# yandex/pire

Hardware: AMD Instinct MI355X
Metric: scanned GB/s (whole node) + ns/byte, 8-regex glued Scanner, 4KiB strings (higher is better)
Workload: dtype u8

## Files before the change

pire_amd/csrc/slow.hip:

```cpp

#include <hip/hip_runtime.h>

#include <algorithm>
#include <cstdio>
#include <cstdlib>
#include <cstring>
#include <memory>
#include <new>
#include <vector>

#include "internal.h"
#include "walk.h"

namespace pirehip {

struct SlowHost {
	uint32_t states = 0, letters = 0, start = 0, words = 0;
	bool empty = false;
	std::vector<uint8_t> letterOf;
	std::vector<uint32_t> masks;
	std::vector<uint32_t> single;
	std::vector<uint32_t> finals;
	std::vector<uint32_t> jumpPos;
	std::vector<uint32_t> jumps;
	bool wide = false;
	std::vector<uint32_t> pair16;
};

struct SlowDevice {
	int device = -1;
	uint8_t* letterOf = nullptr;
	uint32_t* masks = nullptr;
	uint32_t* single = nullptr;
	uint32_t* finals = nullptr;
	uint32_t* jumpPos = nullptr;
	uint32_t* jumps = nullptr;
	uint32_t* pair16 = nullptr;
};

constexpr uint32_t kSlowNone = 0xFFFFFFFFu;
constexpr uint32_t kSlowMulti = 0xFFFFFFFEu;

}

struct pire_hip_slow_table {
	pirehip::SlowHost host;
	pirehip::SlowDevice devs[pirehip::kMaxDevices];
	std::mutex uploadMutex;
};

namespace pirehip {

struct SlowParams {
	const uint8_t* letterOf;
	const uint32_t* masks;
	const uint32_t* single;
	const uint32_t* finals;
	const uint32_t* jumpPos;
	const uint32_t* jumps;
	const uint32_t* pair16;
	uint32_t* overflow;
	const uint32_t* order;
	uint32_t serpentine;
	uint32_t* scratch;
	uint32_t states, letters, start, words, flags, masksInLds, singleInLds;
	const uint8_t* text;
	const uint64_t* offsets;
	uint64_t n, len, stride;
	uint8_t* outFinal;
	uint32_t* outBits;
	unsigned long long* outCounts;
};

template <int K>
__device__ __forceinline__ void SlowStep(const uint32_t* masks, uint32_t letters, uint32_t (&cur)[K], uint32_t letter)
{
	uint32_t next[K];
#pragma unroll
	for (int k = 0; k < K; ++k)
		next[k] = 0;
#pragma unroll
	for (int w = 0; w < K; ++w) {
		uint32_t bits = cur[w];
		while (bits) {
			const uint32_t s = w * 32 + __builtin_ctz(bits);
			bits &= bits - 1;
			const uint32_t* row = masks + (size_t(s) * letters + letter) * K;
#pragma unroll
			for (int k = 0; k < K; ++k)
				next[k] |= row[k];
		}
	}
#pragma unroll
	for (int k = 0; k < K; ++k)
		cur[k] = next[k];
}

template <int K>
struct SlowLane {
	uint32_t lst[4];
	uint32_t cur[K];
	uint32_t E;
	bool bits;

	__device__ __forceinline__ void Start(uint32_t start, uint32_t states)
	{
		E = states;
		lst[0] = start;
		lst[1] = lst[2] = lst[3] = E;
		bits = false;
#pragma unroll
		for (int k = 0; k < K; ++k)
			cur[k] = 0;
	}
	__device__ __forceinline__ void ListToBits()
	{
#pragma unroll
		for (int k = 0; k < K; ++k)
			cur[k] = 0;
#pragma unroll
		for (int i = 0; i < 4; ++i) {
			const uint32_t s = lst[i];
			if (s != E) {
#pragma unroll
				for (int k = 0; k < K; ++k)
					cur[k] |= (s >> 5) == uint32_t(k) ? (1u << (s & 31)) : 0u;
			}
		}
		bits = true;
	}
	__device__ __forceinline__ void BitsToListIfSmall()
	{
		uint32_t count = 0;
#pragma unroll
		for (int k = 0; k < K; ++k)
			count += __popc(cur[k]);
		if (count > 4)
			return;
		uint32_t n[4] = {E, E, E, E};
		uint32_t used = 0;
#pragma unroll
		for (int k = 0; k < K; ++k) {
			uint32_t b = cur[k];
			while (b) {
				const uint32_t s = uint32_t(k) * 32 + __builtin_ctz(b);
				b &= b - 1;
				n[0] = used == 0 ? s : n[0];
				n[1] = used == 1 ? s : n[1];
				n[2] = used == 2 ? s : n[2];
				n[3] = used == 3 ? s : n[3];
				++used;
			}
		}
#pragma unroll
		for (int i = 0; i < 4; ++i)
			lst[i] = n[i];
		bits = false;
	}
	__device__ __forceinline__ void Step(const uint32_t* masks, const uint2* single, uint32_t letters, uint32_t letter)
	{
		if (!bits) {
			uint32_t n[4], extra = 0, extras = 0, multi = 0;
#pragma unroll
			for (int i = 0; i < 4; ++i) {
				const uint2 r = single[__umul24(lst[i], letters) + letter];
				n[i] = r.x;
				multi |= r.x;
				const bool has = int32_t(r.y) >= 0;
				extra = has ? r.y : extra;
				extras += has ? 1u : 0u;
			}
			uint32_t overflow = multi >> 31;
			if (__any(extras != 0)) {
				overflow |= uint32_t(extras > 1);
				uint32_t placed = uint32_t(extras != 1);
#pragma unroll
				for (int j = 0; j < 4; ++j) {
					const uint32_t take = uint32_t(n[j] == E) & (placed ^ 1u);
					n[j] = take ? extra : n[j];
					placed |= take;
				}
				overflow |= placed ^ 1u;
			}
			if (!overflow) {
#pragma unroll
				for (int i = 0; i < 4; ++i)
					lst[i] = n[i];
				return;
			}
			ListToBits();
		}
		SlowStep<K>(masks, letters, cur, letter);
		BitsToListIfSmall();
	}
	__device__ __forceinline__ bool Final(const uint32_t* finals) const
	{
		bool fin = false;
		if (bits) {
#pragma unroll
			for (int k = 0; k < K; ++k)
				fin = fin || (cur[k] & finals[k]) != 0;
		} else {
#pragma unroll
			for (int i = 0; i < 4; ++i)
				fin = fin || (lst[i] != E && ((finals[lst[i] >> 5] >> (lst[i] & 31)) & 1u));
		}
		return fin;
	}
};

template <int K>
__global__ __launch_bounds__(1024) void SlowScanKernel(SlowParams p)
{
	extern __shared__ __attribute__((aligned(16))) uint8_t lds[];
	uint8_t* ldsLetter = lds;
	uint32_t* ldsSingle = reinterpret_cast<uint32_t*>(lds + 272);
	const uint32_t entries = p.states * p.letters;
	const uint32_t singleEntries = (p.states + 1) * p.letters;
	uint32_t* ldsMasks = ldsSingle + (p.singleInLds ? 2 * singleEntries : 0);
	for (uint32_t i = threadIdx.x; i < 264; i += blockDim.x)
		ldsLetter[i] = p.letterOf[i];
	if (p.singleInLds)
		for (uint32_t i = threadIdx.x; i < 2 * singleEntries; i += blockDim.x)
			ldsSingle[i] = p.single[i];
	const uint32_t maskWords = entries * K;
	if (p.masksInLds)
		for (uint32_t i = threadIdx.x; i < maskWords; i += blockDim.x)
			ldsMasks[i] = p.masks[i];
	__syncthreads();
	const uint32_t* masks = p.masksInLds ? ldsMasks : p.masks;
	const uint2* single = reinterpret_cast<const uint2*>(p.singleInLds ? ldsSingle : p.single);

	const uint64_t stride = uint64_t(gridDim.x) * blockDim.x;
	unsigned long long finals = 0, strings = 0;
	const uint64_t todo = p.overflow ? p.overflow[0] : p.n;
	for (uint64_t k = uint64_t(blockIdx.x) * blockDim.x + threadIdx.x; k < todo; k += stride) {
		const uint64_t s = p.overflow ? p.overflow[1 + k] : k;
		uint64_t b, e;
		if (p.offsets) {
			b = p.offsets[s];
			e = p.offsets[s + 1];
		} else {
			b = s * p.stride;
			e = b + p.len;
		}
		SlowLane<K> lane;
		lane.Start(p.start, p.states);
		if (p.flags & PIRE_HIP_RUN_BEGIN)
			lane.Step(masks, single, p.letters, ldsLetter[kBeginMark]);
		const uint8_t* ptr = p.text + b;
		const uint8_t* end = p.text + e;
		for (; ptr < end && (reinterpret_cast<uintptr_t>(ptr) & 15); ++ptr)
			lane.Step(masks, single, p.letters, ldsLetter[*ptr]);
		uint4 ahead = ptr + 16 <= end ? *reinterpret_cast<const uint4*>(ptr) : uint4{0, 0, 0, 0};
		for (; ptr + 16 <= end; ptr += 16) {
			uint4 v = ahead;
			if (ptr + 32 <= end)
				ahead = *reinterpret_cast<const uint4*>(ptr + 16);
#pragma unroll 1
			for (int i = 0; i < 16; ++i) {
				lane.Step(masks, single, p.letters, ldsLetter[v.x & 0xFF]);
				NextByte(v);
			}
		}
		for (; ptr < end; ++ptr)
			lane.Step(masks, single, p.letters, ldsLetter[*ptr]);
		if (p.flags & PIRE_HIP_RUN_END)
			lane.Step(masks, single, p.letters, ldsLetter[kEndMark]);
		const bool fin = lane.Final(p.finals);
		if (p.outFinal)
			p.outFinal[s] = fin ? 1 : 0;
		if (p.outBits) {
			if (!lane.bits)
				lane.ListToBits();
#pragma unroll
			for (int k = 0; k < K; ++k)
				if (uint32_t(k) < p.words)
					p.outBits[s * p.words + k] = lane.cur[k];
		}
		finals += fin ? 1 : 0;
		strings += 1;
	}
	if (p.outCounts) {
		for (int off = 32; off > 0; off >>= 1) {
			finals += __shfl_down(finals, off);
			strings += __shfl_down(strings, off);
		}
		if ((threadIdx.x & 63) == 0 && strings) {
			atomicAdd(&p.outCounts[0], finals);
			atomicAdd(&p.outCounts[1], strings);
		}
	}
}

constexpr int kListSlots = 16;
constexpr uint32_t kListMulti = 0x7FFFu;
constexpr uint32_t kListMaxRows = 16383;

typedef const __attribute__((address_space(3))) uint32_t* LdsWordPtr;

template <int T>
__device__ __forceinline__ void ListStepT(uint32_t tabBase, uint32_t letter4, uint32_t (&lst)[kListSlots], bool& ovf)
{
	constexpr int N = 4 * T;
	uint32_t r[N];
	uint32_t sumHi = 0;
	const uint32_t base = letter4 + tabBase;
#pragma unroll
	for (int i = 0; i < N; ++i) {
		uint32_t addr;
		asm("v_mad_u32_u16 %0, %1, 1, %2" : "=v"(addr) : "v"(lst[i]), "v"(base));
		r[i] = *reinterpret_cast<LdsWordPtr>(static_cast<uintptr_t>(addr));
		sumHi += r[i] >> 16;
	}
	const bool spawn = sumHi != 0;
	const uint32_t extra = sumHi & 0x7FFFu;
	bool over = sumHi >= (0x8000u | kListMulti);
	if (N == kListSlots)
		over = over || (spawn && (r[N - 1] & 0xFFFFu) != 0);
	if (__any(over)) {
		ovf = ovf || over;
#pragma unroll
		for (int i = 0; i < N; ++i)
			r[i] = over ? 0u : r[i];
	}
	const bool shift = spawn && !ovf;
	if (N < kListSlots)
		lst[N] = shift ? r[N - 1] : 0u;
#pragma unroll
	for (int i = N - 1; i > 0; --i)
		lst[i] = shift ? r[i - 1] : r[i];
	lst[0] = shift ? extra << 2 : r[0];
}

__device__ __forceinline__ uint32_t ListTop(const uint32_t (&lst)[kListSlots])
{
	uint32_t top = 1;
#pragma unroll
	for (int g = 1; g < kListSlots / 4; ++g)
		top = __any((lst[4 * g] | lst[4 * g + 1] | lst[4 * g + 2] | lst[4 * g + 3]) != 0) ? uint32_t(g + 1) : top;
	return top;
}

__device__ __forceinline__ void ListStepTop(uint32_t tabBase, uint32_t letter4, uint32_t (&lst)[kListSlots], bool& ovf, uint32_t& top)
{
	switch (top) {
	case 1:
		ListStepT<1>(tabBase, letter4, lst, ovf);
		top = __any(lst[4] != 0) ? 2u : 1u;
		break;
	case 2:
		ListStepT<2>(tabBase, letter4, lst, ovf);
		top = __any(lst[8] != 0) ? 3u : __any((lst[4] | lst[5] | lst[6] | lst[7]) != 0) ? 2u : 1u;
		break;
	case 3:
		ListStepT<3>(tabBase, letter4, lst, ovf);
		top = __any(lst[12] != 0) ? 4u : __any((lst[8] | lst[9] | lst[10] | lst[11]) != 0) ? 3u : 2u;
		break;
	default:
		ListStepT<4>(tabBase, letter4, lst, ovf);
		top = __any((lst[12] | lst[13] | lst[14] | lst[15]) != 0) ? 4u : 3u;
		break;
	}
}

__device__ __forceinline__ void ListStep(uint32_t tabBase, uint32_t letter4, uint32_t (&lst)[kListSlots], bool& ovf)
{
	ListStepT<kListSlots / 4>(tabBase, letter4, lst, ovf);
}

__global__ __launch_bounds__(1024) void SlowListKernel(SlowParams p)
{
	extern __shared__ __attribute__((aligned(16))) uint8_t lds[];
	uint8_t* ldsLetter = lds;
	uint32_t* tab = reinterpret_cast<uint32_t*>(lds + 1056 + 16);
	const uint32_t tabBase = 1056 + 16;
	uint32_t* ldsLetter4 = reinterpret_cast<uint32_t*>(lds);
	const uint32_t entries = (p.states + 1) * p.letters;
	for (uint32_t i = threadIdx.x; i < 264; i += blockDim.x)
		ldsLetter4[i] = 4u * p.letterOf[i];
	for (uint32_t i = threadIdx.x; i < entries; i += blockDim.x)
		tab[i] = p.pair16[i];
	__syncthreads();
	(void)ldsLetter;
	const uint64_t stride = uint64_t(gridDim.x) * blockDim.x;
	unsigned long long finals = 0, strings = 0;
	for (uint64_t pass = 0; pass * stride < p.n; ++pass) {
		const uint64_t k = OrderedIndex(pass, uint64_t(blockIdx.x) * blockDim.x + threadIdx.x, stride, p.serpentine != 0);
		if (k >= p.n)
			continue;
		const uint64_t s = p.order ? p.order[k] : k;
		uint64_t b, e;
		if (p.offsets) {
			b = p.offsets[s];
			e = p.offsets[s + 1];
		} else {
#if defined(PIRE_EXP) && PIRE_EXP == 21
			b = (s & 63) * p.stride;
#else
			b = s * p.stride;
#endif
			e = b + p.len;
		}
		uint32_t lst[kListSlots];
		lst[0] = (p.start + 1) * p.letters * 4;
#pragma unroll
		for (int i = 1; i < kListSlots; ++i)
			lst[i] = 0;
		bool ovf = false;
		if (p.flags & PIRE_HIP_RUN_BEGIN)
			ListStep(tabBase, ldsLetter4[kBeginMark], lst, ovf);
		const uint8_t* ptr = p.text + b;
		const uint8_t* end = p.text + e;
		for (; ptr < end && (reinterpret_cast<uintptr_t>(ptr) & 15); ++ptr)
			ListStep(tabBase, ldsLetter4[*ptr], lst, ovf);
		uint4 ahead = ptr + 16 <= end ? *reinterpret_cast<const uint4*>(ptr) : uint4{0, 0, 0, 0};
		uint32_t top = ListTop(lst);
		for (; ptr + 16 <= end; ptr += 16) {
			top = __builtin_amdgcn_readfirstlane(top);
			uint4 v = ahead;
			if (ptr + 32 <= end)
				ahead = *reinterpret_cast<const uint4*>(ptr + 16);
#pragma unroll 1
			for (int i = 0; i < 4; ++i) {
				const uint32_t x = v.x;
				ListStepTop(tabBase, ldsLetter4[x & 0xFF], lst, ovf, top);
				ListStepTop(tabBase, ldsLetter4[(x >> 8) & 0xFF], lst, ovf, top);
				ListStepTop(tabBase, ldsLetter4[(x >> 16) & 0xFF], lst, ovf, top);
				ListStepTop(tabBase, ldsLetter4[x >> 24], lst, ovf, top);
				v.x = v.y;
				v.y = v.z;
				v.z = v.w;
			}
		}
		for (; ptr < end; ++ptr)
			ListStep(tabBase, ldsLetter4[*ptr], lst, ovf);
		if (p.flags & PIRE_HIP_RUN_END)
			ListStep(tabBase, ldsLetter4[kEndMark], lst, ovf);
		if (ovf) {
			const uint32_t k = atomicAdd(&p.overflow[0], 1u);
			p.overflow[1 + k] = uint32_t(s);
			continue;
		}
		bool fin = false;
#pragma unroll
		for (int i = 0; i < kListSlots; ++i) {
			const uint32_t row = (lst[i] & 0xFFFFu) >> 2;
			lst[i] = row ? row / p.letters - 1 : p.states;
			fin = fin || (lst[i] != p.states && ((p.finals[lst[i] >> 5] >> (lst[i] & 31)) & 1u));
		}
		if (p.outFinal)
			p.outFinal[s] = fin ? 1 : 0;
		if (p.outBits) {
			uint32_t* row = p.outBits + s * p.words;
			for (uint32_t w = 0; w < p.words; ++w) {
				uint32_t v = 0;
#pragma unroll
				for (int i = 0; i < kListSlots; ++i)
					v |= (lst[i] != p.states && (lst[i] >> 5) == w) ? 1u << (lst[i] & 31) : 0u;
				row[w] = v;
			}
		}
		finals += fin ? 1 : 0;
		strings += 1;
	}
	if (p.outCounts) {
		for (int off = 32; off > 0; off >>= 1) {
			finals += __shfl_down(finals, off);
			strings += __shfl_down(strings, off);
		}
		if ((threadIdx.x & 63) == 0 && strings) {
			atomicAdd(&p.outCounts[0], finals);
			atomicAdd(&p.outCounts[1], strings);
		}
	}
}

template <bool SETS_LDS>
__device__ __forceinline__ void WideSync()
{
	if (SETS_LDS)
		__builtin_amdgcn_fence(__ATOMIC_SEQ_CST, "workgroup");
	else
		__builtin_amdgcn_fence(__ATOMIC_SEQ_CST, "agent");
	__builtin_amdgcn_wave_barrier();
}
template <bool SETS_LDS>
__device__ __forceinline__ uint32_t WideLoad(const uint32_t* q)
{
	if (SETS_LDS)
		return *q;
	return __hip_atomic_load(q, __ATOMIC_RELAXED, __HIP_MEMORY_SCOPE_AGENT);
}
template <bool SETS_LDS>
__device__ __forceinline__ void WideStore(uint32_t* q, uint32_t v)
{
	if (SETS_LDS)
		*q = v;
	else
		__hip_atomic_store(q, v, __ATOMIC_RELAXED, __HIP_MEMORY_SCOPE_AGENT);
}

struct WideTables {
	const uint32_t* pos;
	const uint32_t* jumps;
};

template <bool SETS_LDS>
__device__ __forceinline__ void WideStep(const SlowParams& p, const WideTables& T, uint32_t*& cur, uint32_t*& next,
                                         uint32_t letter, uint32_t lane)
{
	for (uint32_t w = lane; w < p.words; w += 64)
		WideStore<SETS_LDS>(&next[w], 0u);
	WideSync<SETS_LDS>();
	for (uint32_t w0 = 0; w0 < p.words; w0 += 64) {
		const uint32_t mine = w0 + lane < p.words ? WideLoad<SETS_LDS>(&cur[w0 + lane]) : 0u;
		unsigned long long nz = __ballot(mine != 0);
		while (nz) {
			const int j = __builtin_ctzll(nz);
			nz &= nz - 1;
			uint32_t bits = uint32_t(__builtin_amdgcn_readlane(int(mine), j));
			const uint32_t base = (w0 + uint32_t(j)) * 32;
			while (bits) {
				const uint32_t s = base + uint32_t(__builtin_ctz(bits));
				bits &= bits - 1;
				const uint32_t* pos = T.pos + size_t(s) * p.letters + letter;
				const uint32_t lo = pos[0], hi = pos[1];
				for (uint32_t k = lo + lane; k < hi; k += 64) {
					const uint32_t t = T.jumps[k];
					atomicOr(&next[t >> 5], 1u << (t & 31));
				}
			}
		}
	}
	WideSync<SETS_LDS>();
	uint32_t* tmp = cur;
	cur = next;
	next = tmp;
}

template <bool SETS_LDS>
__global__ __launch_bounds__(1024) void SlowWideKernel(SlowParams p, uint32_t wavesPerBlock, uint32_t posInLds,
                                                       uint32_t jumpsInLds, uint32_t njumps)
{
	extern __shared__ __attribute__((aligned(16))) uint8_t lds[];
	uint8_t* ldsLetter = lds;
	uint32_t* ldsPos = reinterpret_cast<uint32_t*>(lds + 272);
	const uint32_t npos = p.states * p.letters + 1;
	uint32_t* ldsJumps = ldsPos + (posInLds ? npos : 0);
	uint32_t* ldsSets = ldsJumps + (jumpsInLds ? njumps : 0);
	for (uint32_t i = threadIdx.x; i < 264; i += blockDim.x)
		ldsLetter[i] = p.letterOf[i];
	if (posInLds)
		for (uint32_t i = threadIdx.x; i < npos; i += blockDim.x)
			ldsPos[i] = p.jumpPos[i];
	if (jumpsInLds)
		for (uint32_t i = threadIdx.x; i < njumps; i += blockDim.x)
			ldsJumps[i] = p.jumps[i];
	__syncthreads();
	WideTables T;
	T.pos = posInLds ? ldsPos : p.jumpPos;
	T.jumps = jumpsInLds ? ldsJumps : p.jumps;
	const uint32_t lane = threadIdx.x & 63;
	const uint32_t wave = threadIdx.x >> 6;
	const uint64_t gwave = uint64_t(blockIdx.x) * wavesPerBlock + wave;
	uint32_t* setA = SETS_LDS ? ldsSets + size_t(wave) * 2 * p.words : p.scratch + gwave * 2 * p.words;
	uint32_t* setB = setA + p.words;
	unsigned long long finals = 0, strings = 0;
	const uint64_t todo = p.overflow ? p.overflow[0] : p.n;
	for (uint64_t k = gwave; k < todo; k += uint64_t(gridDim.x) * wavesPerBlock) {
		const uint64_t s = p.overflow ? p.overflow[1 + k] : k;
		uint64_t b, e;
		if (p.offsets) {
			b = p.offsets[s];
			e = p.offsets[s + 1];
		} else {
			b = s * p.stride;
			e = b + p.len;
		}
		uint32_t *cur = setA, *next = setB;
		for (uint32_t w = lane; w < p.words; w += 64)
			WideStore<SETS_LDS>(&cur[w], (p.start >> 5) == w ? 1u << (p.start & 31) : 0u);
		WideSync<SETS_LDS>();
		if (p.flags & PIRE_HIP_RUN_BEGIN)
			WideStep<SETS_LDS>(p, T, cur, next, ldsLetter[kBeginMark], lane);
		for (uint64_t i = b; i < e; i += 64) {
			const uint32_t mine = i + lane < e ? p.text[i + lane] : 0u;
			const uint32_t cnt = e - i < 64 ? uint32_t(e - i) : 64u;
			for (uint32_t k = 0; k < cnt; ++k)
				WideStep<SETS_LDS>(p, T, cur, next, ldsLetter[__builtin_amdgcn_readlane(int(mine), int(k))], lane);
		}
		if (p.flags & PIRE_HIP_RUN_END)
			WideStep<SETS_LDS>(p, T, cur, next, ldsLetter[kEndMark], lane);
		bool fin = false;
		for (uint32_t w = lane; w < p.words; w += 64) {
			const uint32_t v = WideLoad<SETS_LDS>(&cur[w]);
			fin = fin || (v & p.finals[w]) != 0;
			if (p.outBits)
				p.outBits[s * p.words + w] = v;
		}
		fin = __any(fin);
		if (p.outFinal && lane == 0)
			p.outFinal[s] = fin ? 1 : 0;
		finals += fin ? 1 : 0;
		strings += 1;
		WideSync<SETS_LDS>();
	}
	if (p.outCounts && lane == 0 && strings) {
		atomicAdd(&p.outCounts[0], finals);
		atomicAdd(&p.outCounts[1], strings);
	}
}

namespace {

size_t Up8(size_t v) { return (v + 7) & ~size_t(7); }

int BadSlow(const char* msg)
{
	SetError(msg);
	return PIRE_HIP_EFORMAT;
}

int BuildSlowHost(const void* blob, size_t len, SlowHost* out)
{
	const uint8_t* p = static_cast<const uint8_t*>(blob);
	if (!p || len < 24 + 24 + 8)
		return BadSlow("EOF reached while reading the SlowScanner header");
	uint32_t hdr[6];
	memcpy(hdr, p, 24);
	if (hdr[0] != 0x45524950u || hdr[2] != 8 || hdr[3] != 16)
		return BadSlow("Serialized regexp incompatible with your system");
	if (hdr[1] != 7 && hdr[1] != 6)
		return BadSlow("You are trying to used an incompatible version of a serialized regexp");
	if (hdr[4] != 3  || hdr[5] != 24)
		return BadSlow("Serialized regexp incompatible with your system");
	uint64_t states, letters, start;
	memcpy(&states, p + 24, 8);
	memcpy(&letters, p + 32, 8);
	memcpy(&start, p + 40, 8);
	size_t pos = 48;
	const bool empty = p[pos] != 0;
	pos += 8;
	SlowHost& h = *out;
	h = SlowHost();
	h.empty = empty;
	if (empty) {
		h.states = 1;
		h.letters = 1;
		h.start = 0;
		h.words = 1;
		h.letterOf.assign(kMaxChar, 0);
		h.masks.assign(1, 0);
		h.single.assign(4, kSlowNone);
		h.single[0] = h.single[2] = 1;
		h.finals.assign(1, 0);
		return PIRE_HIP_OK;
	}
	if (states == 0 || letters == 0 || letters > 256 || states > (1u << 20) || start >= states)
		return BadSlow("Corrupt SlowScanner: bad geometry");
	h.states = uint32_t(states);
	h.letters = uint32_t(letters);
	h.start = uint32_t(start);
	h.words = (h.states + 31) / 32;
	if (len < pos + size_t(kMaxChar) * 8)
		return BadSlow("EOF reached while reading SlowScanner letters");
	h.letterOf.assign(kMaxChar, 0);
	for (uint32_t c = 0; c < kMaxChar; ++c) {
		uint64_t v;
		memcpy(&v, p + pos + size_t(c) * 8, 8);
		if (v >= letters)
			return BadSlow("Corrupt SlowScanner: letter out of range");
		h.letterOf[c] = uint8_t(v);
	}
	pos += size_t(kMaxChar) * 8;
	if (len < pos + Up8(states))
		return BadSlow("EOF reached while reading SlowScanner finals");
	h.finals.assign(h.words, 0);
	for (uint32_t s = 0; s < h.states; ++s)
		if (p[pos + s])
			h.finals[s >> 5] |= 1u << (s & 31);
	pos += Up8(states);
	const size_t npos = size_t(states) * letters + 1;
	if (len < pos + npos * 8)
		return BadSlow("EOF reached while reading SlowScanner jump positions");
	std::vector<uint64_t> jumpPos(npos);
	memcpy(jumpPos.data(), p + pos, npos * 8);
	pos += npos * 8;
	const uint64_t njumps = jumpPos[npos - 1];
	if (len < pos + Up8(size_t(njumps) * 4))
		return BadSlow("EOF reached while reading SlowScanner jumps");
	if (njumps >= (1ull << 32))
		return BadSlow("Corrupt SlowScanner: too many jumps");
	for (size_t i = 0; i + 1 < npos; ++i)
		if (jumpPos[i] > jumpPos[i + 1] || jumpPos[i + 1] > njumps)
			return BadSlow("Corrupt SlowScanner: jump positions not monotone");
	for (uint64_t k = 0; k < njumps; ++k) {
		uint32_t tgt;
		memcpy(&tgt, p + pos + size_t(k) * 4, 4);
		if (tgt >= states)
			return BadSlow("Corrupt SlowScanner: jump target out of range");
	}
	if ((size_t(states) + 1) * letters <= kListMaxRows) {
		h.pair16.assign((size_t(states) + 1) * letters, 0);
		for (size_t i = 0; i + 1 < npos; ++i) {
			const uint32_t self = uint32_t(i / letters);
			uint32_t t0 = kSlowNone, t1 = kSlowNone;
			bool multi = false;
			for (uint64_t k = jumpPos[i]; k < jumpPos[i + 1]; ++k) {
				uint32_t tgt;
				memcpy(&tgt, p + pos + size_t(k) * 4, 4);
				if (t0 == kSlowNone)
					t0 = tgt;
				else if (tgt == t0)
					continue;
				else if (t1 == kSlowNone)
					t1 = tgt;
				else if (tgt != t1)
					multi = true;
			}
			if (t1 != kSlowNone && t0 == self)
				std::swap(t0, t1);
			const auto rowIndex = [&](uint32_t t) { return uint32_t((size_t(t) + 1) * letters); };
			uint32_t& w = h.pair16[letters + i];
			if (multi)
				w = (1u << 31) | (kListMulti << 16);
			else if (t1 != kSlowNone)
				w = (1u << 31) | (rowIndex(t1) << 16) | (rowIndex(t0) * 4);
			else if (t0 != kSlowNone)
				w = rowIndex(t0) * 4;
		}
	}
	h.wide = h.words > 8;
	if (h.wide) {
		h.jumpPos.resize(npos);
		for (size_t i = 0; i < npos; ++i)
			h.jumpPos[i] = uint32_t(jumpPos[i]);
		h.jumps.resize(size_t(njumps));
		memcpy(h.jumps.data(), p + pos, size_t(njumps) * 4);
		return PIRE_HIP_OK;
	}
	h.masks.assign(size_t(states) * letters * h.words, 0);
	for (size_t i = 0; i + 1 < npos; ++i)
		for (uint64_t k = jumpPos[i]; k < jumpPos[i + 1]; ++k) {
			uint32_t tgt;
			memcpy(&tgt, p + pos + size_t(k) * 4, 4);
			h.masks[i * h.words + (tgt >> 5)] |= 1u << (tgt & 31);
		}
	h.single.assign(size_t(states + 1) * letters * 2, kSlowNone);
	for (uint64_t l = 0; l < letters; ++l)
		h.single[(size_t(states) * letters + l) * 2] = uint32_t(states);
	for (size_t i = 0; i + 1 < npos; ++i) {
		uint32_t t0 = kSlowNone, t1 = kSlowNone;
		bool multi = false;
		for (uint64_t k = jumpPos[i]; k < jumpPos[i + 1]; ++k) {
			uint32_t tgt;
			memcpy(&tgt, p + pos + size_t(k) * 4, 4);
			if (t0 == kSlowNone)
				t0 = tgt;
			else if (tgt == t0)
				continue;
			else if (t1 == kSlowNone)
				t1 = tgt;
			else if (tgt != t1)
				multi = true;
		}
		h.single[2 * i] = multi ? kSlowMulti : t0 == kSlowNone ? uint32_t(states) : t0;
		h.single[2 * i + 1] = multi ? kSlowNone : t1;
	}
	return PIRE_HIP_OK;
}

template <class T>
int PutSlow(T** dst, const std::vector<T>& src)
{
	*dst = nullptr;
	hipError_t e = hipMalloc(reinterpret_cast<void**>(dst), std::max<size_t>(src.size() * sizeof(T), 16));
	if (e != hipSuccess)
		return HipFail(e, "hipMalloc(slow table)");
	if (!src.empty()) {
		e = hipMemcpy(*dst, src.data(), src.size() * sizeof(T), hipMemcpyHostToDevice);
		if (e != hipSuccess)
			return HipFail(e, "hipMemcpy(slow table)");
	}
	return PIRE_HIP_OK;
}

void FreeSlowDevice(SlowDevice* d)
{
	if (d->device < 0)
		return;
	if (d->letterOf) (void)hipFree(d->letterOf);
	if (d->masks) (void)hipFree(d->masks);
	if (d->single) (void)hipFree(d->single);
	if (d->finals) (void)hipFree(d->finals);
	if (d->jumpPos) (void)hipFree(d->jumpPos);
	if (d->jumps) (void)hipFree(d->jumps);
	if (d->pair16) (void)hipFree(d->pair16);
	*d = SlowDevice();
}

int DeviceK(uint32_t words)
{
	return words <= 1 ? 1 : words <= 2 ? 2 : words <= 4 ? 4 : words <= 8 ? 8 : 0;
}

int UploadSlow(pire_hip_slow_table* t, SlowDevice* image)
{
	std::lock_guard<std::mutex> lock(t->uploadMutex);
	int dev = -1;
	hipError_t e = hipGetDevice(&dev);
	if (e != hipSuccess)
		return HipFail(e, "hipGetDevice");
	if (dev < 0 || dev >= kMaxDevices) {
		SetError("HIP device ordinal out of range");
		return PIRE_HIP_EUNSUPPORTED;
	}
	if (t->devs[dev].device == dev) {
		*image = t->devs[dev];
		return PIRE_HIP_OK;
	}
	const SlowHost& h = t->host;
	if (h.wide) {
		SlowDevice d;
		int rc;
		if ((rc = PutSlow(&d.letterOf, h.letterOf)) || (rc = PutSlow(&d.finals, h.finals)) ||
		    (rc = PutSlow(&d.jumpPos, h.jumpPos)) || (rc = PutSlow(&d.jumps, h.jumps)) ||
		    (!h.pair16.empty() && (rc = PutSlow(&d.pair16, h.pair16)))) {
			d.device = dev;
			FreeSlowDevice(&d);
			return rc;
		}
		d.device = dev;
		t->devs[dev] = d;
		*image = d;
		return PIRE_HIP_OK;
	}
	const int K = DeviceK(h.words);
	std::vector<uint32_t> masks(size_t(h.states) * h.letters * K, 0), finals(K, 0);
	for (size_t i = 0; i < size_t(h.states) * h.letters; ++i)
		for (uint32_t w = 0; w < h.words; ++w)
			masks[i * K + w] = h.masks[i * h.words + w];
	for (uint32_t w = 0; w < h.words; ++w)
		finals[w] = h.finals[w];
	SlowDevice d;
	int rc;
	if ((rc = PutSlow(&d.letterOf, h.letterOf)) || (rc = PutSlow(&d.masks, masks)) || (rc = PutSlow(&d.single, h.single)) ||
	    (rc = PutSlow(&d.finals, finals)) || (!h.pair16.empty() && (rc = PutSlow(&d.pair16, h.pair16)))) {
		d.device = dev;
		FreeSlowDevice(&d);
		return rc;
	}
	d.device = dev;
	t->devs[dev] = d;
	*image = d;
	return PIRE_HIP_OK;
}

struct SlowGeometry {
	uint32_t states, letters, words, njumps;
	bool listTable;
};

struct SlowGrid {
	uint32_t threads = 0, blocks = 0, ldsBytes = 0;
	uint64_t passes = 0;
};

enum : uint32_t { kSlowFirstList = 0, kSlowFirstScan = 1, kSlowFirstWide = 2 };

struct SlowPlan {
	uint32_t first = 0;
	uint32_t walker = 0;
	uint32_t K = 0;
	uint32_t listTable = 0;
	uint32_t byLength = 0;
	SlowGrid list;
	uint32_t singleInLds = 0, masksInLds = 0;
	uint32_t waves = 0, posInLds = 0, jumpsInLds = 0, setsInLds = 0;
	SlowGrid walk;
};

constexpr size_t kSlowSingleLdsMax = 64 * 1024;
constexpr size_t kSlowTablesLdsMax = 150 * 1024;
constexpr uint64_t kSlowScanBigBatch = 128 * 1024;
constexpr size_t kSlowWideLdsRoom = 158 * 1024 - 272;
constexpr uint32_t kSlowWideWaves = 16;

uint64_t GridPasses(uint64_t n, uint64_t lanes)
{
	return (n + lanes - 1) / lanes;
}

SlowPlan PlanSlow(const SlowGeometry& g, uint64_t n, bool ragged, int cus, const pire_hip_config& c)
{
	SlowPlan plan;
	const bool wide = g.words > 8;
	plan.K = wide ? 0 : uint32_t(DeviceK(g.words));
	plan.listTable = g.listTable ? 1 : 0;
	plan.walker = wide ? kSlowFirstWide : kSlowFirstScan;
	plan.first = g.listTable && n < (1ull << 32) - 1 && !c.slow_no_list ? uint32_t(kSlowFirstList) : plan.walker;
	if (plan.first == kSlowFirstList) {
		plan.byLength = ragged && OrdersByLength(n, c) ? 1 : 0;
		SlowGrid& l = plan.list;
		l.ldsBytes = uint32_t(1056 + 16 + size_t(g.states + 1) * g.letters * 4);
		l.threads = n >= uint64_t(cus) * 2048 ? 1024 : n >= uint64_t(cus) * 512 ? 512 : 256;
		l.blocks = GridBlocks(n, cus, l.threads, l.ldsBytes);
		l.passes = GridPasses(n, uint64_t(l.blocks) * l.threads);
	}
	SlowGrid& w = plan.walk;
	if (!wide) {
		const size_t maskBytes = size_t(g.states) * g.letters * plan.K * 4;
		const size_t singleBytes = size_t(g.states + 1) * g.letters * 8;
		plan.singleInLds = singleBytes <= kSlowSingleLdsMax ? 1 : 0;
		plan.masksInLds = maskBytes + (plan.singleInLds ? singleBytes : 0) <= kSlowTablesLdsMax ? 1 : 0;
		w.ldsBytes = uint32_t(272 + (plan.singleInLds ? singleBytes : 0) + (plan.masksInLds ? maskBytes : 0));
		w.threads = n >= kSlowScanBigBatch ? 1024 : 256;
		w.blocks = GridBlocks(n, cus, w.threads, w.ldsBytes);
		w.passes = GridPasses(n, uint64_t(w.blocks) * w.threads);
		return plan;
	}
	const size_t setBytes = size_t(g.words) * 8;
	uint32_t waves = uint32_t(std::min<size_t>(kSlowWideWaves, kSlowWideLdsRoom / setBytes));
	const bool inLds = waves >= 1 && !c.slow_sets_in_memory;
	if (!inLds)
		waves = kSlowWideWaves;
	size_t room = kSlowWideLdsRoom - (inLds ? waves * setBytes : 0);
	const size_t posBytes = (size_t(g.states) * g.letters + 1) * 4, jumpBytes = size_t(g.njumps) * 4;
	plan.posInLds = posBytes <= room ? 1 : 0;
	if (plan.posInLds)
		room -= posBytes;
	plan.jumpsInLds = plan.posInLds && jumpBytes <= room ? 1 : 0;
	plan.setsInLds = inLds ? 1 : 0;
	plan.waves = waves;
	w.threads = waves * 64;
	w.blocks = uint32_t(std::max<uint64_t>(1, std::min<uint64_t>((n + waves - 1) / waves, uint64_t(cus))));
	w.ldsBytes = uint32_t(272 + (inLds ? waves * setBytes : 0) + (plan.posInLds ? posBytes : 0) + (plan.jumpsInLds ? jumpBytes : 0));
	w.passes = GridPasses(n, uint64_t(w.blocks) * waves);
	return plan;
}

SlowGeometry GeometryOf(const SlowHost& h)
{
	return SlowGeometry{h.states, h.letters, h.words, uint32_t(h.jumps.size()), !h.pair16.empty()};
}

template <int K>
int LaunchSlowK(const SlowParams& p0, const SlowPlan& plan, hipStream_t stream)
{
	SlowParams p = p0;
	p.singleInLds = plan.singleInLds;
	p.masksInLds = plan.masksInLds;
	return Launch(SlowScanKernel<K>, plan.walk.blocks, plan.walk.threads, plan.walk.ldsBytes, stream, "slow kernel launch", p);
}

int LaunchSlowWide(const SlowParams& p0, const SlowPlan& plan, uint32_t njumps, hipStream_t stream)
{
	SlowParams p = p0;
	StreamScratch scratch(stream);
	if (!plan.setsInLds) {
		if (int rc = scratch.Alloc(uint64_t(plan.walk.blocks) * plan.waves * p.words * 8, "hipMallocAsync(slow scanner sets)"))
			return rc;
		p.scratch = scratch.as<uint32_t>();
	}
	return Launch(plan.setsInLds ? SlowWideKernel<true> : SlowWideKernel<false>, plan.walk.blocks, plan.walk.threads, plan.walk.ldsBytes,
	              stream, "slow kernel launch", p, plan.waves, plan.posInLds, plan.jumpsInLds, njumps);
}

template <class Fallback>
int LaunchSlowListThen(const SlowParams& p0, const SlowPlan& plan, hipStream_t stream, Fallback fallback)
{
	SlowParams p = p0;
	StreamScratch list(stream);
	if (int rc = OverflowList(list, p.n, stream, "hipMallocAsync(slow scanner overflow list)", &p.overflow))
		return rc;
	StreamScratch orderScratch(stream);
	p.order = nullptr;
	if (plan.byLength)
		if (int rc = OrderByLength(p.offsets, p.n, stream, orderScratch, &p.order, &p.serpentine))
			return rc;
	if (int rc = Launch(SlowListKernel, plan.list.blocks, plan.list.threads, plan.list.ldsBytes, stream, "slow kernel launch", p))
		return rc;
	if (GetConfig().slow_stats) {
		uint32_t over = 0;
		if (hipStreamSynchronize(stream) == hipSuccess && hipMemcpy(&over, list.get(), 4, hipMemcpyDeviceToHost) == hipSuccess)
			fprintf(stderr, "pire_hip slow: %u of %llu strings left the list kernel for the %s one\n", over,
			        static_cast<unsigned long long>(p.n), p.words > 8 ? "wave-per-string" : "bitset");
	}
	return fallback(p);
}

int RunSlow(const char* who, pire_hip_slow_table* t, const void* text, const uint64_t* offsets, uint64_t n, uint64_t len, uint64_t stride,
            uint32_t flags, uint8_t* outFinal, uint32_t* outBits, uint64_t* outCounts, const FinalSelectOut* sel, void* streamPtr)
{
	if (!t) {
		SetError(sel ? std::string(who) + ": null table" : std::string("null table"));
		return PIRE_HIP_EINVAL;
	}
	const bool onDevice = (flags & PIRE_HIP_RUN_ON_DEVICE) != 0;
	std::optional<FinalSelectStage> pass;
	if (sel) {
		if (int rc = FinalSelectArgsInvalid(who, n, true, *sel))
			return rc;
		pass.emplace(*sel, onDevice);
		if (n == 0)
			return pass->Empty(static_cast<hipStream_t>(streamPtr));
	}
	SlowDevice image;
	if (int rc = UploadSlow(t, &image))
		return rc;
	hipStream_t stream = static_cast<hipStream_t>(streamPtr);
	const SlowHost& h = t->host;
	SlowParams p;
	memset(&p, 0, sizeof(p));
	p.letterOf = image.letterOf;
	p.masks = image.masks;
	p.single = image.single;
	p.finals = image.finals;
	p.jumpPos = image.jumpPos;
	p.jumps = image.jumps;
	p.pair16 = image.pair16;
	p.states = h.states;
	p.letters = h.letters;
	p.start = h.start;
	p.words = h.words;
	p.flags = flags;
	p.n = n;
	p.len = len;
	p.stride = stride;
	if (n == 0)
		return PIRE_HIP_OK;
	int cus = 0;
	if (int rc = DeviceCUs(&cus))
		return rc;
	const SlowPlan plan = PlanSlow(GeometryOf(h), n, offsets != nullptr, cus, GetConfig());
	auto plain = [&](const SlowParams& q) {
		switch (plan.K) {
		case 0: return LaunchSlowWide(q, plan, uint32_t(h.jumps.size()), stream);
		case 1: return LaunchSlowK<1>(q, plan, stream);
		case 2: return LaunchSlowK<2>(q, plan, stream);
		case 4: return LaunchSlowK<4>(q, plan, stream);
		default: return LaunchSlowK<8>(q, plan, stream);
		}
	};
	auto launch = [&](const SlowParams& q) {
		if (plan.first == kSlowFirstList) {
			NoteKernel("slow_list", "pirehip::SlowListKernel");
			return LaunchSlowListThen(q, plan, stream, plain);
		}
		if (plan.first == kSlowFirstWide)
			NoteKernel("slow_wide", "pirehip::SlowWideKernel");
		else
			NoteKernel("slow", plan.K == 1 ? "pirehip::SlowScanKernel<1>" : plan.K == 2 ? "pirehip::SlowScanKernel<2>" :
			                    plan.K == 4 ? "pirehip::SlowScanKernel<4>" : "pirehip::SlowScanKernel<8>");
		return plain(q);
	};
	BatchIO io(stream, onDevice);
	const unsigned long long* dCnt = nullptr;
	int rc = io.Text(text, offsets, n, len, stride, &p.text, &p.offsets);
	if (!rc && outCounts) {
		rc = io.In(reinterpret_cast<const unsigned long long*>(outCounts), 2, &dCnt);
		p.outCounts = const_cast<unsigned long long*>(dCnt);
	}
	if (!rc && (outFinal || pass))
		rc = io.Result(outFinal, n, n, &p.outFinal);
	if (!rc && outBits)
		rc = io.Result(outBits, n * h.words, n * h.words, &p.outBits);
	io.CopyBack(outCounts, dCnt, 16);
	StreamScratch ownFinal(stream);
	if (!rc && pass) {
		if (!p.outFinal) {
			if ((rc = ownFinal.Alloc(size_t(n), "hipMallocAsync(slow scanner final flags)")))
				return rc;
			p.outFinal = ownFinal.as<uint8_t>();
		}
		rc = pass->Results(io, n);
	}
	if (rc || (rc = io.Ready()) || (rc = launch(p)))
		return rc;
	if (pass && (rc = pass->Launch(p.outFinal, n, stream)))
		return rc;
	if ((rc = io.Finish()))
		return rc;
	return pass ? pass->Back() : PIRE_HIP_OK;
}

}
}

using namespace pirehip;

extern "C" {

int pire_hip_slow_table_create(const void* save_blob, size_t len, pire_hip_slow_table** out)
try {
	if (!out) {
		SetError("null out pointer");
		return PIRE_HIP_EINVAL;
	}
	*out = nullptr;
	std::unique_ptr<pire_hip_slow_table> t(new (std::nothrow) pire_hip_slow_table);
	if (!t) {
		SetError("out of memory");
		return PIRE_HIP_ENOMEM;
	}
	if (int rc = BuildSlowHost(save_blob, len, &t->host))
		return rc;
	*out = t.release();
	return PIRE_HIP_OK;
} catch (...) {
	return pirehip::HandleException();
}

void pire_hip_slow_table_destroy(pire_hip_slow_table* t)
{
	if (!t)
		return;
	int cur = -1;
	(void)hipGetDevice(&cur);
	for (int k = 0; k < kMaxDevices; ++k)
		if (t->devs[k].device >= 0) {
			(void)hipSetDevice(k);
			FreeSlowDevice(&t->devs[k]);
		}
	if (cur >= 0)
		(void)hipSetDevice(cur);
	delete t;
}

int pire_hip_slow_table_get_info(const pire_hip_slow_table* t, pire_hip_slow_info* out)
try {
	if (!t || !out) {
		SetError("null argument");
		return PIRE_HIP_EINVAL;
	}
	memset(out, 0, sizeof(*out));
	out->states = t->host.states;
	out->letters = t->host.letters;
	out->start = t->host.start;
	out->words = t->host.words;
	out->empty = t->host.empty ? 1 : 0;
	out->mask_bytes = uint64_t(t->host.masks.size()) * 4;
	return PIRE_HIP_OK;
} catch (...) {
	return pirehip::HandleException();
}

int pire_hip_slow_table_plan(const pire_hip_slow_table* t, uint64_t n, uint32_t ragged, uint32_t cus, uint32_t out[24])
try {
	if (!t || !out) {
		SetError("null argument");
		return PIRE_HIP_EINVAL;
	}
	int units = int(cus);
	if (cus == 0)
		if (int rc = DeviceCUs(&units))
			return rc;
	if (units <= 0) {
		SetError("bad CU count");
		return PIRE_HIP_EINVAL;
	}
	const SlowPlan plan = PlanSlow(GeometryOf(t->host), n, ragged != 0, units, GetConfig());
	const SlowGrid& first = plan.first == kSlowFirstList ? plan.list : plan.walk;
	const auto sat = [](uint64_t v) { return uint32_t(std::min<uint64_t>(v, 0xFFFFFFFFu)); };
	memset(out, 0, 24 * sizeof(uint32_t));
	out[0] = plan.first;
	out[1] = plan.walker;
	out[2] = plan.K;
	out[3] = plan.listTable;
	out[4] = plan.singleInLds;
	out[5] = plan.masksInLds;
	out[6] = first.threads;
	out[7] = first.blocks;
	out[8] = first.ldsBytes;
	out[9] = sat(first.passes);
	out[10] = plan.waves;
	out[11] = plan.posInLds;
	out[12] = plan.jumpsInLds;
	out[13] = plan.setsInLds;
	out[14] = plan.byLength;
	out[15] = plan.walk.threads;
	out[16] = plan.walk.blocks;
	out[17] = plan.walk.ldsBytes;
	out[18] = sat(plan.walk.passes);
	out[19] = uint32_t(units);
	return PIRE_HIP_OK;
} catch (...) {
	return pirehip::HandleException();
}

int pire_hip_slow_run(pire_hip_slow_table* t, const void* text, const uint64_t* offsets, uint64_t n, uint32_t flags,
                      uint8_t* out_final, uint32_t* out_state_bits, uint64_t* out_counts, void* stream)
try {
	if (n && !offsets) {
		SetError("null offsets");
		return PIRE_HIP_EINVAL;
	}
	return RunSlow("pire_hip_slow_run", t, text, offsets, n, 0, 0, flags, out_final, out_state_bits, out_counts, nullptr, stream);
} catch (...) {
	return pirehip::HandleException();
}

int pire_hip_slow_run_strided(pire_hip_slow_table* t, const void* text, uint64_t n, uint64_t len, uint64_t stride,
                              uint32_t flags, uint8_t* out_final, uint32_t* out_state_bits, uint64_t* out_counts,
                              void* stream)
try {
	if (stride < len) {
		SetError("stride smaller than len");
		return PIRE_HIP_EINVAL;
	}
	return RunSlow("pire_hip_slow_run_strided", t, text, nullptr, n, len, stride, flags, out_final, out_state_bits, out_counts, nullptr, stream);
} catch (...) {
	return pirehip::HandleException();
}

int pire_hip_slow_run_select(pire_hip_slow_table* t, const void* text, const uint64_t* offsets, uint64_t n, uint32_t flags, uint32_t mode,
                             uint8_t* out_final, uint32_t* out_state_bits, uint64_t* out_counts, uint64_t* out_hits, uint64_t hit_cap,
                             uint64_t* out_hit_count, void* stream)
try {
	if (n && !offsets) {
		SetError("pire_hip_slow_run_select: null offsets");
		return PIRE_HIP_EINVAL;
	}
	const FinalSelectOut sel = {mode, out_hits, hit_cap, out_hit_count};
	return RunSlow("pire_hip_slow_run_select", t, text, offsets, n, 0, 0, flags, out_final, out_state_bits, out_counts, &sel, stream);
} catch (...) {
	return pirehip::HandleException();
}

int pire_hip_slow_run_select_strided(pire_hip_slow_table* t, const void* text, uint64_t n, uint64_t len, uint64_t stride, uint32_t flags,
                                     uint32_t mode, uint8_t* out_final, uint32_t* out_state_bits, uint64_t* out_counts, uint64_t* out_hits,
                                     uint64_t hit_cap, uint64_t* out_hit_count, void* stream)
try {
	if (stride < len) {
		SetError("pire_hip_slow_run_select_strided: stride smaller than len");
		return PIRE_HIP_EINVAL;
	}
	const FinalSelectOut sel = {mode, out_hits, hit_cap, out_hit_count};
	return RunSlow("pire_hip_slow_run_select_strided", t, text, nullptr, n, len, stride, flags, out_final, out_state_bits, out_counts, &sel,
	               stream);
} catch (...) {
	return pirehip::HandleException();
}

}
```

Before: 6546.

## Restructure list-DFA inner loop into top-specialized runs with prefetched letter lookups

```diff
diff --git a/pire_amd/csrc/slow.hip b/pire_amd/csrc/slow.hip
--- a/pire_amd/csrc/slow.hip
+++ b/pire_amd/csrc/slow.hip
@@ -7,6 +7,7 @@
 #include <cstring>
 #include <memory>
 #include <new>
+#include <type_traits>
 #include <vector>
 
 #include "internal.h"
@@ -299,90 +300,97 @@
 
 typedef const __attribute__((address_space(3))) uint32_t* LdsWordPtr;
 
-template <int T>
-__device__ __forceinline__ void ListStepT(uint32_t tabBase, uint32_t letter4, uint32_t (&lst)[kListSlots], bool& ovf)
+template <int B, int E, class F>
+__device__ __forceinline__ void StaticFor(F&& f)
+{
+	if constexpr (B < E) {
+		f(std::integral_constant<int, B>());
+		StaticFor<B + 1, E>(f);
+	}
+}
+
+template <int T, class F>
+__device__ __forceinline__ void ListStepT(uint32_t letter4, uint32_t (&lst)[kListSlots], uint32_t& ovf, F&& ahead)
 {
 	constexpr int N = 4 * T;
 	uint32_t r[N];
 	uint32_t sumHi = 0;
-	const uint32_t base = letter4 + tabBase;
-#pragma unroll
-	for (int i = 0; i < N; ++i) {
+	StaticFor<0, N>([&](auto i) {
 		uint32_t addr;
-		asm("v_mad_u32_u16 %0, %1, 1, %2" : "=v"(addr) : "v"(lst[i]), "v"(base));
+		asm("v_mad_u32_u16 %0, %1, 1, %2" : "=v"(addr) : "v"(lst[i]), "v"(letter4));
 		r[i] = *reinterpret_cast<LdsWordPtr>(static_cast<uintptr_t>(addr));
 		sumHi += r[i] >> 16;
-	}
-	const bool spawn = sumHi != 0;
-	const uint32_t extra = sumHi & 0x7FFFu;
+	});
+	ahead();
 	bool over = sumHi >= (0x8000u | kListMulti);
 	if (N == kListSlots)
-		over = over || (spawn && (r[N - 1] & 0xFFFFu) != 0);
+		over = over || (sumHi != 0 && (r[N - 1] & 0xFFFFu) != 0);
 	if (__any(over)) {
-		ovf = ovf || over;
-#pragma unroll
-		for (int i = 0; i < N; ++i)
-			r[i] = over ? 0u : r[i];
-	}
-	const bool shift = spawn && !ovf;
-	if (N < kListSlots)
+		ovf = over ? 1u : ovf;
+		StaticFor<0, N>([&](auto i) { r[i] = over ? 0u : r[i]; });
+		sumHi = over ? 0u : sumHi;
+	}
+	const bool shift = sumHi != 0;
+	if constexpr (N < kListSlots)
 		lst[N] = shift ? r[N - 1] : 0u;
-#pragma unroll
-	for (int i = N - 1; i > 0; --i)
-		lst[i] = shift ? r[i - 1] : r[i];
-	lst[0] = shift ? extra << 2 : r[0];
+	StaticFor<1, N>([&](auto i) {
+		constexpr int I = N - decltype(i)::value;
+		lst[I] = shift ? r[I - 1] : r[I];
+	});
+	lst[0] = shift ? sumHi << 2 : r[0];
 }
 
 __device__ __forceinline__ uint32_t ListTop(const uint32_t (&lst)[kListSlots])
 {
 	uint32_t top = 1;
-#pragma unroll
-	for (int g = 1; g < kListSlots / 4; ++g)
-		top = __any((lst[4 * g] | lst[4 * g + 1] | lst[4 * g + 2] | lst[4 * g + 3]) != 0) ? uint32_t(g + 1) : top;
+	StaticFor<1, kListSlots / 4>([&](auto g) {
+		constexpr int G = decltype(g)::value;
+		top = __any((lst[4 * G] | lst[4 * G + 1] | lst[4 * G + 2] | lst[4 * G + 3]) != 0) ? uint32_t(G + 1) : top;
+	});
 	return top;
 }
 
-__device__ __forceinline__ void ListStepTop(uint32_t tabBase, uint32_t letter4, uint32_t (&lst)[kListSlots], bool& ovf, uint32_t& top)
-{
-	switch (top) {
-	case 1:
-		ListStepT<1>(tabBase, letter4, lst, ovf);
-		top = __any(lst[4] != 0) ? 2u : 1u;
-		break;
-	case 2:
-		ListStepT<2>(tabBase, letter4, lst, ovf);
-		top = __any(lst[8] != 0) ? 3u : __any((lst[4] | lst[5] | lst[6] | lst[7]) != 0) ? 2u : 1u;
-		break;
-	case 3:
-		ListStepT<3>(tabBase, letter4, lst, ovf);
-		top = __any(lst[12] != 0) ? 4u : __any((lst[8] | lst[9] | lst[10] | lst[11]) != 0) ? 3u : 2u;
-		break;
-	default:
-		ListStepT<4>(tabBase, letter4, lst, ovf);
-		top = __any((lst[12] | lst[13] | lst[14] | lst[15]) != 0) ? 4u : 3u;
-		break;
-	}
-}
-
-__device__ __forceinline__ void ListStep(uint32_t tabBase, uint32_t letter4, uint32_t (&lst)[kListSlots], bool& ovf)
-{
-	ListStepT<kListSlots / 4>(tabBase, letter4, lst, ovf);
+template <int T>
+__device__ __forceinline__ void ListRun(const uint32_t* ldsLetter4, const uint4& v, uint32_t after, uint32_t& x, uint32_t& q,
+                                        uint32_t& letter4, uint32_t (&lst)[kListSlots], uint32_t& ovf, uint32_t& top)
+{
+	constexpr int N = 4 * T;
+#pragma clang loop unroll(disable)
+	do {
+		if ((q & 31) == 0)
+			x = q == 32 ? v.y : q == 64 ? v.z : q == 96 ? v.w : after;
+		uint32_t next;
+		ListStepT<T>(letter4, lst, ovf, [&]() { next = ldsLetter4[(x >> (q & 31)) & 0xFF]; });
+		letter4 = next;
+		q += 8;
+		if constexpr (T == 1)
+			top = __any(lst[N] != 0) ? 2u : 1u;
+		else if constexpr (T < kListSlots / 4)
+			top = __any(lst[N] != 0)                                             ? uint32_t(T + 1)
+			      : __any((lst[N - 4] | lst[N - 3] | lst[N - 2] | lst[N - 1]) != 0) ? uint32_t(T)
+			                                                                        : uint32_t(T - 1);
+		else
+			top = __any((lst[N - 4] | lst[N - 3] | lst[N - 2] | lst[N - 1]) != 0) ? uint32_t(T) : uint32_t(T - 1);
+	} while (top == uint32_t(T) && q <= 128);
+}
+
+__device__ __forceinline__ void ListStep(uint32_t letter4, uint32_t (&lst)[kListSlots], uint32_t& ovf)
+{
+	ListStepT<kListSlots / 4>(letter4, lst, ovf, []() {});
 }
 
 __global__ __launch_bounds__(1024) void SlowListKernel(SlowParams p)
 {
 	extern __shared__ __attribute__((aligned(16))) uint8_t lds[];
-	uint8_t* ldsLetter = lds;
 	uint32_t* tab = reinterpret_cast<uint32_t*>(lds + 1056 + 16);
 	const uint32_t tabBase = 1056 + 16;
 	uint32_t* ldsLetter4 = reinterpret_cast<uint32_t*>(lds);
 	const uint32_t entries = (p.states + 1) * p.letters;
 	for (uint32_t i = threadIdx.x; i < 264; i += blockDim.x)
-		ldsLetter4[i] = 4u * p.letterOf[i];
+		ldsLetter4[i] = 4u * p.letterOf[i] + tabBase;
 	for (uint32_t i = threadIdx.x; i < entries; i += blockDim.x)
 		tab[i] = p.pair16[i];
 	__syncthreads();
-	(void)ldsLetter;
 	const uint64_t stride = uint64_t(gridDim.x) * blockDim.x;
 	unsigned long long finals = 0, strings = 0;
 	for (uint64_t pass = 0; pass * stride < p.n; ++pass) {
@@ -404,60 +412,65 @@
 		}
 		uint32_t lst[kListSlots];
 		lst[0] = (p.start + 1) * p.letters * 4;
-#pragma unroll
-		for (int i = 1; i < kListSlots; ++i)
-			lst[i] = 0;
-		bool ovf = false;
+		StaticFor<1, kListSlots>([&](auto i) { lst[i] = 0; });
+		uint32_t ovf = 0;
 		if (p.flags & PIRE_HIP_RUN_BEGIN)
-			ListStep(tabBase, ldsLetter4[kBeginMark], lst, ovf);
+			ListStep(ldsLetter4[kBeginMark], lst, ovf);
 		const uint8_t* ptr = p.text + b;
 		const uint8_t* end = p.text + e;
 		for (; ptr < end && (reinterpret_cast<uintptr_t>(ptr) & 15); ++ptr)
-			ListStep(tabBase, ldsLetter4[*ptr], lst, ovf);
+			ListStep(ldsLetter4[*ptr], lst, ovf);
 		uint4 ahead = ptr + 16 <= end ? *reinterpret_cast<const uint4*>(ptr) : uint4{0, 0, 0, 0};
 		uint32_t top = ListTop(lst);
+		uint32_t letter4 = ldsLetter4[ahead.x & 0xFF];
 		for (; ptr + 16 <= end; ptr += 16) {
 			top = __builtin_amdgcn_readfirstlane(top);
 			uint4 v = ahead;
 			if (ptr + 32 <= end)
 				ahead = *reinterpret_cast<const uint4*>(ptr + 16);
-#pragma unroll 1
-			for (int i = 0; i < 4; ++i) {
-				const uint32_t x = v.x;
-				ListStepTop(tabBase, ldsLetter4[x & 0xFF], lst, ovf, top);
-				ListStepTop(tabBase, ldsLetter4[(x >> 8) & 0xFF], lst, ovf, top);
-				ListStepTop(tabBase, ldsLetter4[(x >> 16) & 0xFF], lst, ovf, top);
-				ListStepTop(tabBase, ldsLetter4[x >> 24], lst, ovf, top);
-				v.x = v.y;
-				v.y = v.z;
-				v.z = v.w;
+			const uint32_t after = ahead.x;
+			uint32_t x = v.x, q = 8;
+			if (top == 1)
+				ListRun<1>(ldsLetter4, v, after, x, q, letter4, lst, ovf, top);
+			while (q <= 128) {
+				switch (top) {
+				case 1:
+					ListRun<1>(ldsLetter4, v, after, x, q, letter4, lst, ovf, top);
+					break;
+				case 2:
+					ListRun<2>(ldsLetter4, v, after, x, q, letter4, lst, ovf, top);
+					break;
+				case 3:
+					ListRun<3>(ldsLetter4, v, after, x, q, letter4, lst, ovf, top);
+					break;
+				default:
+					ListRun<4>(ldsLetter4, v, after, x, q, letter4, lst, ovf, top);
+					break;
+				}
 			}
 		}
 		for (; ptr < end; ++ptr)
-			ListStep(tabBase, ldsLetter4[*ptr], lst, ovf);
+			ListStep(ldsLetter4[*ptr], lst, ovf);
 		if (p.flags & PIRE_HIP_RUN_END)
-			ListStep(tabBase, ldsLetter4[kEndMark], lst, ovf);
+			ListStep(ldsLetter4[kEndMark], lst, ovf);
 		if (ovf) {
 			const uint32_t k = atomicAdd(&p.overflow[0], 1u);
 			p.overflow[1 + k] = uint32_t(s);
 			continue;
 		}
 		bool fin = false;
-#pragma unroll
-		for (int i = 0; i < kListSlots; ++i) {
+		StaticFor<0, kListSlots>([&](auto i) {
 			const uint32_t row = (lst[i] & 0xFFFFu) >> 2;
 			lst[i] = row ? row / p.letters - 1 : p.states;
 			fin = fin || (lst[i] != p.states && ((p.finals[lst[i] >> 5] >> (lst[i] & 31)) & 1u));
-		}
+		});
 		if (p.outFinal)
 			p.outFinal[s] = fin ? 1 : 0;
 		if (p.outBits) {
 			uint32_t* row = p.outBits + s * p.words;
 			for (uint32_t w = 0; w < p.words; ++w) {
 				uint32_t v = 0;
-#pragma unroll
-				for (int i = 0; i < kListSlots; ++i)
-					v |= (lst[i] != p.states && (lst[i] >> 5) == w) ? 1u << (lst[i] & 31) : 0u;
+				StaticFor<0, kListSlots>([&](auto i) { v |= (lst[i] != p.states && (lst[i] >> 5) == w) ? 1u << (lst[i] & 31) : 0u; });
 				row[w] = v;
 			}
 		}
```

Result: no change. 6536 (median of 3 runs) (-0.1%).
